# mueller-franzes/medfusion

Measured on AMD Instinct MI355X. Metric: images/sec at 256x256, 150 DDIM steps (DiffusionPipeline.sample incl. VAE decode), higher is better.
Workload: dtype f32 (emulated: fp16 pairs -- 23-bit operands, and 23-bit STORAGE of the tensors between the UNet's conv blocks: they exist as fp16 pairs only)

## Files before the change

### medfusion_amd/csrc/conv_f16x2.h

```cpp
#pragma once
#include "common.h"
#include "split_f16.h"

#ifndef MFC2_HZ
#define MFC2_HZ 0
#endif
#ifndef MFC2_OUT_STORE
#define MFC2_OUT_STORE 0
#endif

namespace mfc2 {
using namespace mf;

typedef float f32x16 __attribute__((ext_vector_type(16)));
typedef float f32x4 __attribute__((ext_vector_type(4)));
typedef unsigned int u32x4 __attribute__((ext_vector_type(4)));
typedef _Float16 f16x8 __attribute__((ext_vector_type(8)));
typedef _Float16 f16x2 __attribute__((ext_vector_type(2)));

struct FuseP {
  int on, act;
  float eps, bconst;
  double count;
  const float* gamma;
  const float* beta;
  const float* res_f32;
  const void* res_pairs;
  const float* res_bound;
  const float* res_slots;
  int res_nslots;
  int tiles_per_sample;
  const float* emb;
  long emb_stride;
  const float* emb_bound;
  float* out_f32;
  void* out_pairs;
  float* out_bound;
  unsigned* rv;
  unsigned* rv_err;
};

struct ConvP2 {
  const void* x1;
  const void* x2;
  const void* w;
  const float* bound1;
  const float* bound2;
  const float* bias;
  int N, Hin, Win, C1, C2, Cin, Cout;
  int Wout, Heff, Weff, KH, KW, stride, pad;
  int M, K, HWout;
  int cgroups, cg_per_split, splitk;
  int tiles_m, tiles_n;
  unsigned bytes1, bytes2, bytesw;
  int subpix, hw_src;
  int wphase_rows;
  int walk_n_fast;
  int tree;
  int wexp;
  int Hout;
  int bound_slots;
  int out_nt;
  float* y;
  float* out_bound;
  long slab;
  double* gn_partial;
  float* handoff;
  unsigned* sync;
  int gn_groups, gn_parts, gn_cpg;
  FuseP fz;
  float wl1_1, wl1_2;
  void* y_pairs;
  float* y_pair_bound;
  float bmax;
#if MFC2_HZ & (256 | 512)
  float* dbg;
#endif
};

static_assert(offsetof(ConvP2, wexp) == 168, "the ramp block: 6 pointers + 30 ints, nothing else in front of wexp");
static_assert(offsetof(ConvP2, gn_groups) - offsetof(ConvP2, wexp) <= 64 && offsetof(ConvP2, fz) + offsetof(FuseP, bconst) - offsetof(ConvP2, gn_groups) <= 64 &&
              offsetof(FuseP, res_nslots) - offsetof(FuseP, bconst) <= 64 && offsetof(FuseP, emb_stride) - offsetof(FuseP, res_nslots) <= 64 &&
              offsetof(ConvP2, wl1_1) - offsetof(ConvP2, fz) - offsetof(FuseP, emb_stride) <= 64 && offsetof(ConvP2, bmax) - offsetof(ConvP2, wl1_1) <= 64,
              "MFC2_RAMP_ARGS touches every 64-byte line of the epilogue's part");

#define MFC2_RAMP_ARGS(P)                                                                                               \
  __builtin_amdgcn_sched_barrier(0);    \
  asm volatile("" : "+s"(P.x1), "+s"(P.x2), "+s"(P.w), "+s"(P.bound1), "+s"(P.bound2), "+s"(P.bias), "+s"(P.N), "+s"(P.Hin), "+s"(P.Win), \
               "+s"(P.C1), "+s"(P.C2), "+s"(P.Cin), "+s"(P.Cout), "+s"(P.Wout));                                        \
  asm volatile("" : "+s"(P.Heff), "+s"(P.Weff), "+s"(P.KH), "+s"(P.KW), "+s"(P.stride), "+s"(P.pad), "+s"(P.M), "+s"(P.K), "+s"(P.HWout), \
               "+s"(P.cgroups), "+s"(P.cg_per_split), "+s"(P.splitk), "+s"(P.tiles_m), "+s"(P.tiles_n));                \
  asm volatile("" : "+s"(P.bytes1), "+s"(P.bytes2), "+s"(P.bytesw), "+s"(P.subpix), "+s"(P.hw_src), "+s"(P.wphase_rows), "+s"(P.walk_n_fast), \
               "+s"(P.tree)                                                                                             \
               : "s"(P.wexp), "s"(P.gn_groups), "s"(__float_as_int(P.fz.bconst)), "s"(P.fz.res_nslots), "s"((int)P.fz.emb_stride), "s"(__float_as_int(P.wl1_1)),   \
                 "s"(__float_as_int(P.bmax)));

__device__ __forceinline__ int xcd_remap2(int bid, int total) {
  const int q = total >> 3, r = total & 7;
  const int xcd = bid & 7, within = bid >> 3;
  const int base = xcd < r ? xcd * (q + 1) : r * (q + 1) + (xcd - r) * q;
  return base + within;
}

#ifndef MFC2_HZ
#define MFC2_HZ 0
#endif
#define MFC2_HZ_ON(BIT) ((MFC2_HZ >> (BIT)) & 1)
#ifndef MFC2_HZ_PAD
#define MFC2_HZ_PAD 7
#endif

__device__ __forceinline__ float hz_add(float a, float b) { float r; asm volatile("v_add_f32 %0, %1, %2" : "=v"(r) : "v"(a), "v"(b)); return r; }
__device__ __forceinline__ float hz_mul(float a, float b) { float r; asm volatile("v_mul_f32 %0, %1, %2" : "=v"(r) : "v"(a), "v"(b)); return r; }

#define MFC2_EPILOGUE_ARGS(OFF)                                                                                         \
  const char __attribute__((address_space(4)))* pk_ =                                                                   \
      (const char __attribute__((address_space(4)))*)__builtin_amdgcn_kernarg_segment_ptr() + (OFF);                    \
  asm volatile("" : "+s"(pk_));                                                                                         \
  const ConvP2& p = *(const ConvP2*)pk_;

#define MFC2_WAIT_VM(N) asm volatile("s_waitcnt vmcnt(%0)" ::"n"(N) : "memory")
#if MFC2_HZ & 512
#define MFC2_STAMP(I) { if (p.dbg && threadIdx.x == 0) reinterpret_cast<unsigned long*>(p.dbg)[(long)MFC2_BID * 8 + (I)] = __builtin_amdgcn_s_memrealtime(); }
#else
#define MFC2_STAMP(I)
#endif
#define MFC2_WAIT_LGKM0() asm volatile("s_waitcnt lgkmcnt(0)" ::: "memory")

#define MFC2_BODY_AS_KERNEL 1
#define MFC2_BID blockIdx.x
#define MFC2_KARG_OFF 0
#include "conv_f16x2_body.inc"
#undef MFC2_BODY_AS_KERNEL
#undef MFC2_BID
#undef MFC2_KARG_OFF
#define MFC2_BODY_AS_KERNEL 0
#define MFC2_BID bid
#define MFC2_KARG_OFF karg_off
#include "conv_f16x2_body.inc"
#undef MFC2_BODY_AS_KERNEL
#undef MFC2_BID
#undef MFC2_KARG_OFF

__global__ __launch_bounds__(256) void split_act_f16x2_kernel(const float* __restrict__ x, u32x4* __restrict__ out, long octets,
                                                              const float* __restrict__ bound, long octets_per_row) {
  const long stride = (long)gridDim.x * blockDim.x;
  for (long o = (long)blockIdx.x * blockDim.x + threadIdx.x; o < octets; o += stride) {
    const float sc = bound ? exp2i(-scale_exp_of(bound[o / octets_per_row])) : 1.f;
    const f32x4 v0 = *reinterpret_cast<const f32x4*>(x + o * 8) * sc, v1 = *reinterpret_cast<const f32x4*>(x + o * 8 + 4) * sc;
    u32x4 hi, lo;
    split8_f16(v0, v1, hi, lo);
    out[o * 2] = hi;
    out[o * 2 + 1] = lo;
  }
}

__global__ __launch_bounds__(256) void split_act_slots_kernel(const float* __restrict__ x, u32x4* __restrict__ out, long octets_per_row,
                                                              const float* __restrict__ slots, int nslots, float* __restrict__ bound_out) {
  __shared__ float sm[4];
  const int row = blockIdx.y, tid = threadIdx.x;
  float m = 0.f;
  for (int i = tid; i < nslots; i += 256) m = fmaxf(m, slots[(long)row * nslots + i]);
  m = mf::wave_max(m);
  if ((tid & 63) == 0) sm[tid >> 6] = m;
  __syncthreads();
  const float b = fmaxf(fmaxf(sm[0], sm[1]), fmaxf(sm[2], sm[3]));
  if (blockIdx.x == 0 && tid == 0) bound_out[row] = b;
  const float sc = exp2i(-scale_exp_of(b));
  const long base = (long)row * octets_per_row;
  for (long o = (long)blockIdx.x * 256 + tid; o < octets_per_row; o += (long)gridDim.x * 256) {
    const f32x4 v0 = *reinterpret_cast<const f32x4*>(x + (base + o) * 8) * sc, v1 = *reinterpret_cast<const f32x4*>(x + (base + o) * 8 + 4) * sc;
    u32x4 hi, lo;
    split8_f16(v0, v1, hi, lo);
    out[(base + o) * 2] = hi;
    out[(base + o) * 2 + 1] = lo;
  }
}

}
```

### medfusion_amd/csrc/conv_f16x2_epilogue.inc

```
  MFC2_WAIT_LGKM0();
  __builtin_amdgcn_s_barrier();
  MFC2_STAMP(4)
  if constexpr (MFC2_HZ_ON(0)) asm volatile("s_nop 15\n\ts_nop 15" ::: "memory");
  if (p.tree) {
#pragma unroll
    for (int i = 0; i < TM; ++i) {
      MFC2_PIXEL_EXPS(i)
      const float f_out = exp2i(last_src2 ? e2_ : e1_) * exp2i(p.wexp);
#pragma unroll
      for (int j = 0; j < TN; ++j)
#pragma unroll
        for (int r = 0; r < 16; ++r) { accm[i][j][r] = (accm[i][j][r] + accx[i][j][r] * kLoInv) * f_out; accx[i][j][r] = 0.f; }
    }
    constexpr int SLOT = BM * BN;
    const int tile = tile_n * p.tiles_m + tile_m;
    float* region = p.handoff + (long)tile * (2L * (p.splitk - 1)) * SLOT;
    const __amdgpu_buffer_rsrc_t rh = __builtin_amdgcn_make_buffer_rsrc(region, 0, (unsigned)(2 * (p.splitk - 1)) * (unsigned)SLOT * 4u, 0x00020000);
    unsigned* cnt = p.sync + (long)tile * (p.splitk - 1);
    unsigned* flag = reinterpret_cast<unsigned*>(smem);
    const unsigned lane_off = (unsigned)((wave * TM * TN * 4) * 64 + lane) * 16u;
    int lbase = 0;
    for (int span = 1; span < p.splitk; span <<= 1) {
      if constexpr (MFC2_HZ_ON(4)) asm volatile("s_nop 15" ::: "memory");
      const int lv = __builtin_ctz(span);
      const int side = (kz >> lv) & 1, pair = kz >> (lv + 1);
      const unsigned mine = (unsigned)(2 * (lbase + pair) + side) * (unsigned)SLOT * 4u, theirs = (unsigned)(2 * (lbase + pair) + (side ^ 1)) * (unsigned)SLOT * 4u;
#pragma unroll
      for (int i = 0; i < TM; ++i)
#pragma unroll
        for (int j = 0; j < TN; ++j)
#pragma unroll
          for (int q = 0; q < 4; ++q) {
            u32x4 v;
#pragma unroll
            for (int e = 0; e < 4; ++e) v[e] = __float_as_uint(accm[i][j][4 * q + e]);
            __builtin_amdgcn_raw_buffer_store_b128(v, rh, lane_off + (unsigned)(((i * TN + j) * 4 + q) * 1024), mine, 0x10);
          }
      MFC2_WAIT_VM(0);
      if constexpr (MFC2_HZ_ON(4)) asm volatile("s_nop 15" ::: "memory");
      __syncthreads();
      if (tid == 0) {
        if (p.tree == 2) {
          __builtin_amdgcn_fence(__ATOMIC_RELEASE, "agent");
          MFC2_WAIT_VM(0);
        }
        const unsigned old = __hip_atomic_fetch_add(cnt + lbase + pair, 1u, __ATOMIC_RELAXED, __HIP_MEMORY_SCOPE_AGENT);
        if (old) __hip_atomic_store(cnt + lbase + pair, 0u, __ATOMIC_RELAXED, __HIP_MEMORY_SCOPE_AGENT);
        if (p.tree == 2 && old) __builtin_amdgcn_fence(__ATOMIC_ACQUIRE, "agent");
        *flag = old;
      }
      __syncthreads();
      const unsigned second = *flag;
      __syncthreads();
      if (!second) return;
      if constexpr (MFC2_HZ_ON(3)) {
        u32x4 pv[TM * TN * 4];
#pragma unroll
        for (int u = 0; u < TM * TN * 4; ++u) pv[u] = __builtin_amdgcn_raw_buffer_load_b128(rh, lane_off + (unsigned)(u * 1024), theirs, 0x10);
        asm volatile("s_waitcnt vmcnt(0)\n\ts_nop 7" ::: "memory");
#if MFC2_HZ & 256
        if (p.dbg) {
          const long plane = (long)p.tiles_m * p.tiles_n * NW * (TM * TN * 16 * 64);
          float* o = p.dbg + ((long)tile * NW + wave) * (TM * TN * 16 * 64) + lane;
#pragma unroll
          for (int u = 0; u < TM * TN * 4; ++u)
#pragma unroll
            for (int e = 0; e < 4; ++e) {
              __builtin_nontemporal_store(accm[u / (4 * TN)][(u / 4) % TN][4 * (u % 4) + e], o + plane + (u * 4 + e) * 64);
              __builtin_nontemporal_store(__uint_as_float(pv[u][e]), o + 2 * plane + (u * 4 + e) * 64);
            }
        }
#endif
#pragma unroll
        for (int u = 0; u < TM * TN * 4; ++u)
#pragma unroll
          for (int e = 0; e < 4; ++e) accm[u / (4 * TN)][(u / 4) % TN][4 * (u % 4) + e] += __uint_as_float(pv[u][e]);
      } else {
#pragma unroll
      for (int i = 0; i < TM; ++i)
#pragma unroll
        for (int j = 0; j < TN; ++j)
#pragma unroll
          for (int q = 0; q < 4; ++q) {
            const u32x4 v = __builtin_amdgcn_raw_buffer_load_b128(rh, lane_off + (unsigned)(((i * TN + j) * 4 + q) * 1024), theirs, 0x10);
#pragma unroll
            for (int e = 0; e < 4; ++e) {
              if constexpr (MFC2_HZ_ON(5)) accm[i][j][4 * q + e] = hz_add(accm[i][j][4 * q + e], __uint_as_float(v[e]));
              else accm[i][j][4 * q + e] += __uint_as_float(v[e]);
            }
          }
      }
      lbase += p.splitk >> (lv + 1);
    }
#if MFC2_HZ & 256
    if (p.dbg) {
      float* o = p.dbg + ((long)tile * NW + wave) * (TM * TN * 16 * 64) + lane;
#pragma unroll
      for (int i = 0; i < TM; ++i)
#pragma unroll
        for (int j = 0; j < TN; ++j)
#pragma unroll
          for (int r = 0; r < 16; ++r) __builtin_nontemporal_store(accm[i][j][r], o + ((i * TN + j) * 16 + r) * 64);
    }
#endif
  }
  MFC2_STAMP(5)
  const bool last_slice = p.splitk == 1 || p.tree;
  constexpr int PITCH = FN * 4 + 16;
  char* stg = smem + wave * (32 * PITCH);
  static_assert(NW * 32 * PITCH <= MFC2_EPILOGUE_LDS_BYTES, "epilogue staging must fit in the pipeline stages");
  constexpr int LPR = FN / 8, RPP = 64 / LPR, NPASS = 32 / RPP;
  const int rr = lane / LPR, c8 = lane % LPR;
  const int col0 = n0 + wn * FN + c8 * 8;
  float* out = p.y + (last_slice ? 0L : (long)kz * p.slab);
#if MFC2_OUT_STORE == 2
  const __amdgpu_buffer_rsrc_t rs_out = __builtin_amdgcn_make_buffer_rsrc(out, 0, (unsigned)((long)p.M * p.Cout * 4), 0x00020000);
#endif
#if MFC2_EXPS_EARLY
  f32x4 b0 = eb0, b1 = eb1;
  asm volatile("" : "+v"(b0), "+v"(b1));
#else
  f32x4 b0 = {0.f, 0.f, 0.f, 0.f}, b1 = {0.f, 0.f, 0.f, 0.f};
  if (last_slice && p.bias) {
    b0 = *reinterpret_cast<const f32x4*>(p.bias + col0);
    b1 = *reinterpret_cast<const f32x4*>(p.bias + col0 + 4);
  }
#endif
  float s1 = 0.f, s2 = 0.f, vmax = 0.f;
  const bool fz = p.fz.on != 0;
  f32x4 yk0[TM][NPASS], yk1[TM][NPASS];
#pragma unroll
  for (int i = 0; i < TM; ++i) {
    MFC2_PIXEL_EXPS(i)
    const float f_out = p.tree ? 1.f : exp2i(last_src2 ? e2_ : e1_) * exp2i(p.wexp);
#pragma unroll
    for (int j = 0; j < TN; ++j)
#pragma unroll
      for (int q = 0; q < 4; ++q) {
        f32x4 v;
#pragma unroll
        for (int e = 0; e < 4; ++e) {
          if constexpr (MFC2_HZ_ON(6)) v[e] = hz_mul(hz_add(accm[i][j][4 * q + e], hz_mul(accx[i][j][4 * q + e], kLoInv)), f_out);
          else v[e] = (accm[i][j][4 * q + e] + accx[i][j][4 * q + e] * kLoInv) * f_out;
        }
        *reinterpret_cast<f32x4*>(stg + (lane & 31) * PITCH + (j * 32 + 8 * q + 4 * fh) * 4) = v;
        if constexpr (MFC2_HZ_ON(7)) asm volatile("s_nop 0" ::: "memory");
        if constexpr (MFC2_HZ_ON(1)) asm volatile("s_nop %1" : "+v"(v) : "n"(MFC2_HZ_PAD) : "memory");
      }
    f32x4 rv0[NPASS], rv1[NPASS];
#pragma unroll
    for (int ps = 0; ps < NPASS; ++ps) {
      rv0[ps] = *reinterpret_cast<const f32x4*>(stg + (ps * RPP + rr) * PITCH + c8 * 32);
      rv1[ps] = *reinterpret_cast<const f32x4*>(stg + (ps * RPP + rr) * PITCH + c8 * 32 + 16);
    }
#pragma unroll
    for (int ps = 0; ps < NPASS; ++ps) {
      const int row = ps * RPP + rr;
      f32x4 v0 = rv0[ps], v1 = rv1[ps];
      if constexpr (MFC2_HZ_ON(2)) asm volatile("s_waitcnt lgkmcnt(0)\n\ts_nop 3" : "+v"(v0), "+v"(v1)::"memory");
      v0 += b0;
      v1 += b1;
      const int m = m0 + wm * FM + i * 32 + row;
      yk0[i][ps] = v0;
      yk1[i][ps] = v1;
      if (fz) {
        if (m < p.M) {
#pragma unroll
          for (int e = 0; e < 4; ++e) {
            s1 += v0[e] + v1[e];
            s2 = fmaf(v0[e], v0[e], s2);
            s2 = fmaf(v1[e], v1[e], s2);
          }
        }
      } else if (m < p.M) {
        long orow = m;
        if (p.subpix) {
          const int n = m / p.HWout, rem = m - n * p.HWout;
          const int ph = rem / p.hw_src, r2 = rem - ph * p.hw_src;
          const int y = r2 / p.Win, x = r2 - y * p.Win;
          orow = ((long)n * p.Hout + 2 * y + (ph >> 1)) * p.Wout + 2 * x + (ph & 1);
        }
#if MFC2_OUT_STORE == 1
        __builtin_nontemporal_store(v0, reinterpret_cast<f32x4*>(out + orow * p.Cout + col0));
        __builtin_nontemporal_store(v1, reinterpret_cast<f32x4*>(out + orow * p.Cout + col0 + 4));
#elif MFC2_OUT_STORE == 2
        {
          const unsigned ob_ = (unsigned)((orow * p.Cout + col0) * 4);
          __builtin_amdgcn_raw_buffer_store_b128(__builtin_bit_cast(u32x4, v0), rs_out, ob_, 0, 0x10);
          __builtin_amdgcn_raw_buffer_store_b128(__builtin_bit_cast(u32x4, v1), rs_out, ob_ + 16u, 0, 0x10);
        }
#else
        if (p.out_nt) {
          __builtin_nontemporal_store(v0, reinterpret_cast<f32x4*>(out + orow * p.Cout + col0));
          __builtin_nontemporal_store(v1, reinterpret_cast<f32x4*>(out + orow * p.Cout + col0 + 4));
        } else {
          *reinterpret_cast<f32x4*>(out + orow * p.Cout + col0) = v0;
          *reinterpret_cast<f32x4*>(out + orow * p.Cout + col0 + 4) = v1;
        }
#endif
        if (p.out_bound) {
#pragma unroll
          for (int e = 0; e < 4; ++e) vmax = fmaxf(vmax, fmaxf(fabsf(v0[e]), fabsf(v1[e])));
        }
        if (p.y_pairs) {
          const int nrow = m / p.HWout;
          const float yb = p.bound1[nrow] * p.wl1_1 + (p.C2 > 0 ? p.bound2[nrow] * p.wl1_2 : 0.f) + p.bmax;
          const float ysc = exp2i(-scale_exp_of(yb));
          sf_u32x4 hi, lo;
          split8_f16<false>(v0 * ysc, v1 * ysc, hi, lo);
          sf_u32x4* op = reinterpret_cast<sf_u32x4*>(reinterpret_cast<char*>(p.y_pairs) + ((orow * p.Cout + col0) >> 3) * 32);
          op[0] = hi;
          op[1] = lo;
          if (m - nrow * p.HWout == 0 && col0 == 0) p.y_pair_bound[nrow] = yb;
        }
#pragma unroll
        for (int e = 0; e < 4; ++e) {
          s1 += v0[e] + v1[e];
          s2 = fmaf(v0[e], v0[e], s2);
          s2 = fmaf(v1[e], v1[e], s2);
        }
      }
    }
  }
  MFC2_STAMP(6)
  const int wm_per_sample = p.HWout >= BM ? WM : p.HWout / FM;
  const int n_first = m0 / p.HWout;
  if (p.out_bound) {
    vmax = wave_max(vmax);
    const int n = n_first + wm / wm_per_sample;
    const int part = p.HWout >= BM ? (m0 - n_first * p.HWout) / BM : 0;
    const int wps = wm_per_sample * WN;
    if (lane == 0 && n < p.N) p.out_bound[(long)n * p.bound_slots + (part * p.tiles_n + tile_n) * wps + (wm % wm_per_sample) * WN + wn] = vmax;
  }
  if (p.gn_partial) {
    double d1 = (double)s1, d2 = (double)s2;
#pragma unroll
    for (int off = LPR; off < 64; off <<= 1) {
      d1 += __shfl_xor(d1, off, 64);
      d2 += __shfl_xor(d2, off, 64);
    }
    __builtin_amdgcn_s_barrier();
    double* red = reinterpret_cast<double*>(smem);
    if (lane < LPR) {
      red[(wave * LPR + lane) * 2] = d1;
      red[(wave * LPR + lane) * 2 + 1] = d2;
    }
    MFC2_WAIT_LGKM0();
    __builtin_amdgcn_s_barrier();
    const int ngl = BN / p.gn_cpg, spt = WM / wm_per_sample;
    if (tid < ngl * spt) {
      const int gl = tid % ngl, si = tid / ngl;
      double s = 0, q = 0;
      const int slots = p.gn_cpg >> 3;
      for (int k = 0; k < slots; ++k) {
        const int slot8 = gl * slots + k;
        const int wn_ = slot8 / LPR, c8_ = slot8 - wn_ * LPR;
        for (int wm_ = si * wm_per_sample; wm_ < (si + 1) * wm_per_sample; ++wm_) {
          const double* d = red + ((wm_ * WN + wn_) * LPR + c8_) * 2;
          s += d[0];
          q += d[1];
        }
      }
      const int n = n_first + si;
      const int part = p.HWout >= BM ? (m0 - n_first * p.HWout) / BM : 0;
      if (n < p.N) {
        double* o = p.gn_partial + (((long)n * p.gn_parts + part) * p.gn_groups + (n0 / p.gn_cpg + gl)) * 2;
        if (fz) {
          __hip_atomic_store(o, s, __ATOMIC_RELAXED, __HIP_MEMORY_SCOPE_AGENT);
          __hip_atomic_store(o + 1, q, __ATOMIC_RELAXED, __HIP_MEMORY_SCOPE_AGENT);
        } else {
          o[0] = s;
          o[1] = q;
        }
      }
    }
  }
  if (fz) {
    MFC2_WAIT_VM(0);
    __syncthreads();
    const int spt = WM / wm_per_sample;
    const int ngl_ = BN / p.gn_cpg;
    const unsigned T_ = (unsigned)p.fz.tiles_per_sample;
    if (tid == 0) {
      for (int si = 0; si < spt; ++si) {
        const int n = n_first + si;
        if (n < p.N) __hip_atomic_fetch_add(p.fz.rv + 2 * n, 1u, __ATOMIC_RELAXED, __HIP_MEMORY_SCOPE_AGENT);
      }
    }
    MFC2_STAMP(6)
    const int si_w = wm / wm_per_sample;
    const int n_w = min(n_first + si_w, p.N - 1);
    float* fzs = reinterpret_cast<float*>(smem + 8192);
    float rb = 0.f;
    if (p.fz.res_slots) {
      for (int si = 0; si < spt; ++si) {
        const int n = min(n_first + si, p.N - 1);
        float mx = 0.f;
        for (int k = tid; k < p.fz.res_nslots; k += NW * 64) mx = fmaxf(mx, p.fz.res_slots[(long)n * p.fz.res_nslots + k]);
        mx = wave_max(mx);
        if (lane == 0) fzs[si * 8 + wave] = mx;
      }
      MFC2_WAIT_LGKM0();
      __syncthreads();
#pragma unroll
      for (int w8 = 0; w8 < NW; ++w8) rb = fmaxf(rb, fzs[si_w * 8 + w8]);
    } else if (p.fz.res_bound) {
      rb = p.fz.res_bound[n_w];
    }
    const float ob_ = p.fz.bconst + rb + (p.fz.emb_bound ? p.fz.emb_bound[n_w] : 0.f);
    const float osc = exp2i(-scale_exp_of(ob_));
    const float rsc = p.fz.res_pairs ? exp2i(scale_exp_of(p.fz.res_bound[n_w])) : 1.f;
    {
      const int part0 = p.HWout >= BM ? (m0 - n_first * p.HWout) / BM : 0;
      if (tile_n == 0 && part0 == 0 && wn == 0 && (wm % wm_per_sample) == 0 && lane == 0 && n_first + si_w < p.N) p.fz.out_bound[n_first + si_w] = ob_;
    }
    f32x4 ga0 = {1.f, 1.f, 1.f, 1.f}, ga1 = ga0, be0 = {0.f, 0.f, 0.f, 0.f}, be1 = be0, em0 = be0, em1 = be0;
    if (p.fz.gamma) {
      ga0 = *reinterpret_cast<const f32x4*>(p.fz.gamma + col0); ga1 = *reinterpret_cast<const f32x4*>(p.fz.gamma + col0 + 4);
      be0 = *reinterpret_cast<const f32x4*>(p.fz.beta + col0);  be1 = *reinterpret_cast<const f32x4*>(p.fz.beta + col0 + 4);
    }
    if (p.fz.emb) {
      const float* er = p.fz.emb + (long)n_w * p.fz.emb_stride + col0;
      em0 = *reinterpret_cast<const f32x4*>(er); em1 = *reinterpret_cast<const f32x4*>(er + 4);
    }
    f32x4 rk0[TM][NPASS], rk1[TM][NPASS];
#pragma unroll
    for (int i = 0; i < TM; ++i)
#pragma unroll
      for (int ps = 0; ps < NPASS; ++ps) {
        const int m = m0 + wm * FM + i * 32 + ps * RPP + rr;
        rk0[i][ps] = f32x4{0.f, 0.f, 0.f, 0.f};
        rk1[i][ps] = f32x4{0.f, 0.f, 0.f, 0.f};
        if (m < p.M) {
          const long e = (long)m * p.Cout + col0;
          if (p.fz.res_pairs) {
            const f32x4* g = reinterpret_cast<const f32x4*>(reinterpret_cast<const char*>(p.fz.res_pairs) + (e >> 3) * 32);
            rk0[i][ps] = g[0]; rk1[i][ps] = g[1];
          } else if (p.fz.res_f32) {
            rk0[i][ps] = *reinterpret_cast<const f32x4*>(p.fz.res_f32 + e); rk1[i][ps] = *reinterpret_cast<const f32x4*>(p.fz.res_f32 + e + 4);
          }
        }
      }
    if (tid == 0) {
      unsigned ok = 1u;
      for (int si = 0; si < spt; ++si) {
        const int n = n_first + si;
        if (n >= p.N) continue;
        const unsigned long t0 = __builtin_amdgcn_s_memrealtime();
        unsigned spins = 0;
        while (__hip_atomic_load(p.fz.rv + 2 * n, __ATOMIC_RELAXED, __HIP_MEMORY_SCOPE_AGENT) < T_) {
          __builtin_amdgcn_s_sleep(1);
          if ((++spins & 127u) == 0u) {
            if (__hip_atomic_load(p.fz.rv_err, __ATOMIC_RELAXED, __HIP_MEMORY_SCOPE_AGENT) != 0u) { ok = 0u; break; }
            if (__builtin_amdgcn_s_memrealtime() - t0 > 5000000ul) {
              __hip_atomic_store(p.fz.rv_err, 1u, __ATOMIC_RELAXED, __HIP_MEMORY_SCOPE_AGENT);
              ok = 0u;
              break;
            }
          }
        }
      }
      reinterpret_cast<unsigned*>(fzs)[64] = ok;
    }
    MFC2_WAIT_LGKM0();
    __syncthreads();
    MFC2_STAMP(7)
    if (tid < ngl_ * spt) {
      const int gl = tid % ngl_, si = tid / ngl_;
      const int n = n_first + si;
      if (n < p.N) {
        const int G_ = p.gn_groups, PPT = 256 / G_, g = n0 / p.gn_cpg + gl;
        double S = 0, Q = 0;
        for (int kk = 0; kk < PPT; ++kk) {
          double a = 0, b = 0;
          for (int k = kk; k < p.gn_parts; k += PPT) {
            const double* r_ = p.gn_partial + (((long)n * p.gn_parts + k) * G_ + g) * 2;
            a += __hip_atomic_load(r_, __ATOMIC_RELAXED, __HIP_MEMORY_SCOPE_AGENT);
            b += __hip_atomic_load(r_ + 1, __ATOMIC_RELAXED, __HIP_MEMORY_SCOPE_AGENT);
          }
          if (kk == 0) { S = a; Q = b; } else { S += a; Q += b; }
        }
        const double mean = S / p.fz.count;
        double var = Q / p.fz.count - mean * mean;
        if (var < 0) var = 0;
        fzs[128 + (si * ngl_ + gl) * 2] = (float)mean;
        fzs[128 + (si * ngl_ + gl) * 2 + 1] = (float)(1.0 / sqrt(var + (double)p.fz.eps));
      }
    }
    MFC2_WAIT_LGKM0();
    __syncthreads();
    if (tid == 0) {
      for (int si = 0; si < spt; ++si) {
        const int n = n_first + si;
        if (n >= p.N) continue;
        const unsigned old = __hip_atomic_fetch_add(p.fz.rv + 2 * n + 1, 1u, __ATOMIC_RELAXED, __HIP_MEMORY_SCOPE_AGENT);
        if (old + 1u == T_) {
          __hip_atomic_store(p.fz.rv + 2 * n, 0u, __ATOMIC_RELAXED, __HIP_MEMORY_SCOPE_AGENT);
          __hip_atomic_store(p.fz.rv + 2 * n + 1, 0u, __ATOMIC_RELAXED, __HIP_MEMORY_SCOPE_AGENT);
        }
      }
    }
    const int glw = (wn * FN + c8 * 8) / p.gn_cpg;
    const float mean_ = fzs[128 + (si_w * ngl_ + glw) * 2], rstd_ = fzs[128 + (si_w * ngl_ + glw) * 2 + 1];
    const bool aff = p.fz.gamma != nullptr, act1 = p.fz.act == 1, resp = p.fz.res_pairs != nullptr, resf = !resp && p.fz.res_f32 != nullptr,
               hasemb = p.fz.emb != nullptr;
#pragma unroll
    for (int i = 0; i < TM; ++i)
#pragma unroll
      for (int ps = 0; ps < NPASS; ++ps) {
        const int m = m0 + wm * FM + i * 32 + ps * RPP + rr;
        if (m < p.M) {
          float ev[8];
#pragma unroll
          for (int e = 0; e < 4; ++e) { ev[e] = yk0[i][ps][e]; ev[4 + e] = yk1[i][ps][e]; }
          const float gv[8] = {ga0[0], ga0[1], ga0[2], ga0[3], ga1[0], ga1[1], ga1[2], ga1[3]};
          const float bv[8] = {be0[0], be0[1], be0[2], be0[3], be1[0], be1[1], be1[2], be1[3]};
          const float mv[8] = {em0[0], em0[1], em0[2], em0[3], em1[0], em1[1], em1[2], em1[3]};
#pragma unroll
          for (int e = 0; e < 8; ++e) {
            float t = (ev[e] - mean_) * rstd_;
            if (aff) t = t * gv[e] + bv[e];
            if (act1) t = swish_apply(t);
            ev[e] = t;
          }
          if (resp) {
            const u32x4 hq = __builtin_bit_cast(u32x4, rk0[i][ps]), lq = __builtin_bit_cast(u32x4, rk1[i][ps]);
#pragma unroll
            for (int e2 = 0; e2 < 4; ++e2) {
              const unsigned hw_ = hq[e2], lw_ = lq[e2];
              const f16x2 h2 = __builtin_bit_cast(f16x2, hw_), l2 = __builtin_bit_cast(f16x2, lw_);
              ev[2 * e2] += ((float)h2[0] + (float)l2[0] * kLoInv) * rsc;
              ev[2 * e2 + 1] += ((float)h2[1] + (float)l2[1] * kLoInv) * rsc;
            }
          } else if (resf) {
#pragma unroll
            for (int e = 0; e < 4; ++e) { ev[e] += rk0[i][ps][e]; ev[4 + e] += rk1[i][ps][e]; }
          }
          if (hasemb) {
#pragma unroll
            for (int e = 0; e < 8; ++e) ev[e] += mv[e];
          }
          const long eo = (long)m * p.Cout + col0;
          if (p.fz.out_f32) {
            *reinterpret_cast<f32x4*>(p.fz.out_f32 + eo) = f32x4{ev[0], ev[1], ev[2], ev[3]};
            *reinterpret_cast<f32x4*>(p.fz.out_f32 + eo + 4) = f32x4{ev[4], ev[5], ev[6], ev[7]};
          }
          sf_u32x4 hi, lo;
          split8_f16<false>(sf_f32x4{ev[0] * osc, ev[1] * osc, ev[2] * osc, ev[3] * osc}, sf_f32x4{ev[4] * osc, ev[5] * osc, ev[6] * osc, ev[7] * osc}, hi, lo);
          sf_u32x4* op = reinterpret_cast<sf_u32x4*>(reinterpret_cast<char*>(p.fz.out_pairs) + (eo >> 3) * 32);
          op[0] = hi;
          op[1] = lo;
        }
      }
  }
```

Baseline: 43.05.

## Restructure conv epilogue drain: preload kernargs, batch LDS staging, prefetch pair bounds

Before the epilogue barrier, the conv epilogue now copies the kernel arguments it uses into scalar/vector registers and preloads the per-row pair-bound values. It stages all TM row-groups through LDS at once when they fit, so the reads are batched instead of serialized per group. Global stores use explicit address_space(1) pointers, and the y_pair_bound writes move to a separate pass after the loop. The aim is to shorten the dependent scalar-load and LDS chains in the drain, at the cost of more registers (pyb/pyn/rv arrays) and possibly lower occupancy.

```diff
diff --git a/medfusion_amd/csrc/conv_f16x2.h b/medfusion_amd/csrc/conv_f16x2.h
--- a/medfusion_amd/csrc/conv_f16x2.h
+++ b/medfusion_amd/csrc/conv_f16x2.h
@@ -113,6 +113,9 @@
 __device__ __forceinline__ float hz_add(float a, float b) { float r; asm volatile("v_add_f32 %0, %1, %2" : "=v"(r) : "v"(a), "v"(b)); return r; }
 __device__ __forceinline__ float hz_mul(float a, float b) { float r; asm volatile("v_mul_f32 %0, %1, %2" : "=v"(r) : "v"(a), "v"(b)); return r; }
 
+#ifndef MFC2_DRAIN_CHAIN
+#define MFC2_DRAIN_CHAIN 2
+#endif
 #define MFC2_EPILOGUE_ARGS(OFF)                                                                                         \
   const char __attribute__((address_space(4)))* pk_ =                                                                   \
       (const char __attribute__((address_space(4)))*)__builtin_amdgcn_kernarg_segment_ptr() + (OFF);                    \
diff --git a/medfusion_amd/csrc/conv_f16x2_epilogue.inc b/medfusion_amd/csrc/conv_f16x2_epilogue.inc
--- a/medfusion_amd/csrc/conv_f16x2_epilogue.inc
+++ b/medfusion_amd/csrc/conv_f16x2_epilogue.inc
@@ -1,12 +1,53 @@
+#if MFC2_DRAIN_CHAIN == 2
+  int dp_M = p.M, dp_Cout = p.Cout, dp_HWout = p.HWout, dp_subpix = p.subpix, dp_out_nt = p.out_nt,
+      dp_fz_on = p.fz.on, dp_hw_src = p.hw_src, dp_Win = p.Win, dp_Hout = p.Hout, dp_Wout = p.Wout;
+  float *dp_y = p.y, *dp_out_bound = p.out_bound;
+  void* dp_y_pairs = p.y_pairs;
+  __builtin_amdgcn_sched_barrier(0);
+  asm volatile("" : "+s"(dp_M), "+s"(dp_Cout), "+s"(dp_HWout), "+s"(dp_subpix), "+s"(dp_out_nt), "+s"(dp_fz_on),
+               "+s"(dp_y), "+s"(dp_out_bound), "+s"(dp_y_pairs));
+  asm volatile("" : "+v"(dp_hw_src), "+v"(dp_Win), "+v"(dp_Hout), "+v"(dp_Wout));
+#define MFC2_G(T, P) ((T __attribute__((address_space(1)))*)(P))
+#define MFC2_DP_SET(F) (dp_##F != nullptr)
+#define dp_slab p.slab
+#define dp_tree p.tree
+#define dp_wexp p.wexp
+#define dp_splitk p.splitk
+#define dp_gn_partial p.gn_partial
+#define MFC2_DP(F) dp_##F
+#else
+#define MFC2_DP(F) p.F
+#define MFC2_DP_SET(F) (p.F != nullptr)
+#define MFC2_G(T, P) (reinterpret_cast<T*>(P))
+#define dp_fz_on p.fz.on
+#endif
+#if MFC2_DRAIN_CHAIN == 2
+  float pyb1[TM][32 / (64 / (FN / 8))] = {}, pyb2[TM][32 / (64 / (FN / 8))] = {};
+  int pyn[TM][32 / (64 / (FN / 8))] = {};
+  float* ypb_ = nullptr;
+  if (MFC2_DP_SET(y_pairs)) {
+    ypb_ = p.y_pair_bound;
+    const float* pb2_ = p.C2 > 0 ? p.bound2 : p.bound1;
+#pragma unroll
+    for (int i = 0; i < TM; ++i)
+#pragma unroll
+      for (int ps = 0; ps < 32 / (64 / (FN / 8)); ++ps) {
+        const int nrow = min(m0 + wm * FM + i * 32 + ps * (64 / (FN / 8)) + lane / (FN / 8), MFC2_DP(M) - 1) / MFC2_DP(HWout);
+        pyn[i][ps] = nrow;
+        pyb1[i][ps] = p.bound1[nrow];
+        pyb2[i][ps] = pb2_[nrow];
+      }
+  }
+#endif
   MFC2_WAIT_LGKM0();
   __builtin_amdgcn_s_barrier();
   MFC2_STAMP(4)
   if constexpr (MFC2_HZ_ON(0)) asm volatile("s_nop 15\n\ts_nop 15" ::: "memory");
-  if (p.tree) {
+  if (MFC2_DP(tree)) {
 #pragma unroll
     for (int i = 0; i < TM; ++i) {
       MFC2_PIXEL_EXPS(i)
-      const float f_out = exp2i(last_src2 ? e2_ : e1_) * exp2i(p.wexp);
+      const float f_out = exp2i(last_src2 ? e2_ : e1_) * exp2i(MFC2_DP(wexp));
 #pragma unroll
       for (int j = 0; j < TN; ++j)
 #pragma unroll
@@ -14,13 +55,13 @@
     }
     constexpr int SLOT = BM * BN;
     const int tile = tile_n * p.tiles_m + tile_m;
-    float* region = p.handoff + (long)tile * (2L * (p.splitk - 1)) * SLOT;
-    const __amdgpu_buffer_rsrc_t rh = __builtin_amdgcn_make_buffer_rsrc(region, 0, (unsigned)(2 * (p.splitk - 1)) * (unsigned)SLOT * 4u, 0x00020000);
-    unsigned* cnt = p.sync + (long)tile * (p.splitk - 1);
+    float* region = p.handoff + (long)tile * (2L * (MFC2_DP(splitk) - 1)) * SLOT;
+    const __amdgpu_buffer_rsrc_t rh = __builtin_amdgcn_make_buffer_rsrc(region, 0, (unsigned)(2 * (MFC2_DP(splitk) - 1)) * (unsigned)SLOT * 4u, 0x00020000);
+    unsigned* cnt = p.sync + (long)tile * (MFC2_DP(splitk) - 1);
     unsigned* flag = reinterpret_cast<unsigned*>(smem);
     const unsigned lane_off = (unsigned)((wave * TM * TN * 4) * 64 + lane) * 16u;
     int lbase = 0;
-    for (int span = 1; span < p.splitk; span <<= 1) {
+    for (int span = 1; span < MFC2_DP(splitk); span <<= 1) {
       if constexpr (MFC2_HZ_ON(4)) asm volatile("s_nop 15" ::: "memory");
       const int lv = __builtin_ctz(span);
       const int side = (kz >> lv) & 1, pair = kz >> (lv + 1);
@@ -40,13 +81,13 @@
       if constexpr (MFC2_HZ_ON(4)) asm volatile("s_nop 15" ::: "memory");
       __syncthreads();
       if (tid == 0) {
-        if (p.tree == 2) {
+        if (MFC2_DP(tree) == 2) {
           __builtin_amdgcn_fence(__ATOMIC_RELEASE, "agent");
           MFC2_WAIT_VM(0);
         }
         const unsigned old = __hip_atomic_fetch_add(cnt + lbase + pair, 1u, __ATOMIC_RELAXED, __HIP_MEMORY_SCOPE_AGENT);
         if (old) __hip_atomic_store(cnt + lbase + pair, 0u, __ATOMIC_RELAXED, __HIP_MEMORY_SCOPE_AGENT);
-        if (p.tree == 2 && old) __builtin_amdgcn_fence(__ATOMIC_ACQUIRE, "agent");
+        if (MFC2_DP(tree) == 2 && old) __builtin_amdgcn_fence(__ATOMIC_ACQUIRE, "agent");
         *flag = old;
       }
       __syncthreads();
@@ -90,7 +131,7 @@
             }
           }
       }
-      lbase += p.splitk >> (lv + 1);
+      lbase += MFC2_DP(splitk) >> (lv + 1);
     }
 #if MFC2_HZ & 256
     if (p.dbg) {
@@ -105,16 +146,18 @@
 #endif
   }
   MFC2_STAMP(5)
-  const bool last_slice = p.splitk == 1 || p.tree;
+  const bool last_slice = MFC2_DP(splitk) == 1 || MFC2_DP(tree);
   constexpr int PITCH = FN * 4 + 16;
-  char* stg = smem + wave * (32 * PITCH);
-  static_assert(NW * 32 * PITCH <= MFC2_EPILOGUE_LDS_BYTES, "epilogue staging must fit in the pipeline stages");
+  constexpr int GI = (MFC2_DRAIN_CHAIN == 2 && NW * TM * 32 * PITCH <= MFC2_EPILOGUE_LDS_BYTES) ? TM : 1;
+  constexpr int STG = GI * 32 * PITCH;
+  char* stg = smem + wave * STG;
+  static_assert(NW * STG <= MFC2_EPILOGUE_LDS_BYTES, "epilogue staging must fit in the pipeline stages");
   constexpr int LPR = FN / 8, RPP = 64 / LPR, NPASS = 32 / RPP;
   const int rr = lane / LPR, c8 = lane % LPR;
   const int col0 = n0 + wn * FN + c8 * 8;
-  float* out = p.y + (last_slice ? 0L : (long)kz * p.slab);
+  float* out = MFC2_DP(y) + (last_slice ? 0L : (long)kz * MFC2_DP(slab));
 #if MFC2_OUT_STORE == 2
-  const __amdgpu_buffer_rsrc_t rs_out = __builtin_amdgcn_make_buffer_rsrc(out, 0, (unsigned)((long)p.M * p.Cout * 4), 0x00020000);
+  const __amdgpu_buffer_rsrc_t rs_out = __builtin_amdgcn_make_buffer_rsrc(out, 0, (unsigned)((long)MFC2_DP(M) * MFC2_DP(Cout) * 4), 0x00020000);
 #endif
 #if MFC2_EXPS_EARLY
   f32x4 b0 = eb0, b1 = eb1;
@@ -127,12 +170,15 @@
   }
 #endif
   float s1 = 0.f, s2 = 0.f, vmax = 0.f;
-  const bool fz = p.fz.on != 0;
+  const bool fz = dp_fz_on != 0;
   f32x4 yk0[TM][NPASS], yk1[TM][NPASS];
-#pragma unroll
-  for (int i = 0; i < TM; ++i) {
+  f32x4 rv0[TM][NPASS], rv1[TM][NPASS];
+#pragma unroll
+  for (int g = 0; g < TM; g += GI) {
+#pragma unroll
+  for (int i = g; i < g + GI; ++i) {
     MFC2_PIXEL_EXPS(i)
-    const float f_out = p.tree ? 1.f : exp2i(last_src2 ? e2_ : e1_) * exp2i(p.wexp);
+    const float f_out = MFC2_DP(tree) ? 1.f : exp2i(last_src2 ? e2_ : e1_) * exp2i(MFC2_DP(wexp));
 #pragma unroll
     for (int j = 0; j < TN; ++j)
 #pragma unroll
@@ -143,20 +189,41 @@
           if constexpr (MFC2_HZ_ON(6)) v[e] = hz_mul(hz_add(accm[i][j][4 * q + e], hz_mul(accx[i][j][4 * q + e], kLoInv)), f_out);
           else v[e] = (accm[i][j][4 * q + e] + accx[i][j][4 * q + e] * kLoInv) * f_out;
         }
-        *reinterpret_cast<f32x4*>(stg + (lane & 31) * PITCH + (j * 32 + 8 * q + 4 * fh) * 4) = v;
+        *reinterpret_cast<f32x4*>(stg + (i - g) * (32 * PITCH) + (lane & 31) * PITCH + (j * 32 + 8 * q + 4 * fh) * 4) = v;
         if constexpr (MFC2_HZ_ON(7)) asm volatile("s_nop 0" ::: "memory");
         if constexpr (MFC2_HZ_ON(1)) asm volatile("s_nop %1" : "+v"(v) : "n"(MFC2_HZ_PAD) : "memory");
       }
-    f32x4 rv0[NPASS], rv1[NPASS];
+  }
+#pragma unroll
+  for (int i = g; i < g + GI; ++i) {
 #pragma unroll
     for (int ps = 0; ps < NPASS; ++ps) {
-      rv0[ps] = *reinterpret_cast<const f32x4*>(stg + (ps * RPP + rr) * PITCH + c8 * 32);
-      rv1[ps] = *reinterpret_cast<const f32x4*>(stg + (ps * RPP + rr) * PITCH + c8 * 32 + 16);
-    }
+      rv0[i][ps] = *reinterpret_cast<const f32x4*>(stg + (i - g) * (32 * PITCH) + (ps * RPP + rr) * PITCH + c8 * 32);
+      rv1[i][ps] = *reinterpret_cast<const f32x4*>(stg + (i - g) * (32 * PITCH) + (ps * RPP + rr) * PITCH + c8 * 32 + 16);
+    }
+  }
+#if MFC2_DRAIN_CHAIN == 2
+  if (g == 0) {
+#pragma unroll
+    for (int i = 0; i < TM; ++i)
+#pragma unroll
+      for (int ps = 0; ps < NPASS; ++ps) asm volatile("" : "+v"(pyb1[i][ps]), "+v"(pyb2[i][ps]));
+    asm volatile("" : "+v"(ypb_));
+    const float wl1_1 = p.wl1_1, wl1_2 = p.wl1_2, bmax = p.bmax;
+    const bool src2 = p.C2 > 0;
+#pragma unroll
+    for (int i = 0; i < TM; ++i)
+#pragma unroll
+      for (int ps = 0; ps < NPASS; ++ps)
+        pyb1[i][ps] = pyb1[i][ps] * wl1_1 + (src2 ? pyb2[i][ps] * wl1_2 : 0.f) + bmax;
+  }
+#endif
+#pragma unroll
+  for (int i = g; i < g + GI; ++i) {
 #pragma unroll
     for (int ps = 0; ps < NPASS; ++ps) {
       const int row = ps * RPP + rr;
-      f32x4 v0 = rv0[ps], v1 = rv1[ps];
+      f32x4 v0 = rv0[i][ps], v1 = rv1[i][ps];
       if constexpr (MFC2_HZ_ON(2)) asm volatile("s_waitcnt lgkmcnt(0)\n\ts_nop 3" : "+v"(v0), "+v"(v1)::"memory");
       v0 += b0;
       v1 += b1;
@@ -164,7 +231,7 @@
       yk0[i][ps] = v0;
       yk1[i][ps] = v1;
       if (fz) {
-        if (m < p.M) {
+        if (m < MFC2_DP(M)) {
 #pragma unroll
           for (int e = 0; e < 4; ++e) {
             s1 += v0[e] + v1[e];
@@ -172,46 +239,52 @@
             s2 = fmaf(v1[e], v1[e], s2);
           }
         }
-      } else if (m < p.M) {
+      } else if (m < MFC2_DP(M)) {
         long orow = m;
-        if (p.subpix) {
-          const int n = m / p.HWout, rem = m - n * p.HWout;
-          const int ph = rem / p.hw_src, r2 = rem - ph * p.hw_src;
-          const int y = r2 / p.Win, x = r2 - y * p.Win;
-          orow = ((long)n * p.Hout + 2 * y + (ph >> 1)) * p.Wout + 2 * x + (ph & 1);
+        if (MFC2_DP(subpix)) {
+          const int n = m / MFC2_DP(HWout), rem = m - n * MFC2_DP(HWout);
+          const int ph = rem / MFC2_DP(hw_src), r2 = rem - ph * MFC2_DP(hw_src);
+          const int y = r2 / MFC2_DP(Win), x = r2 - y * MFC2_DP(Win);
+          orow = ((long)n * MFC2_DP(Hout) + 2 * y + (ph >> 1)) * MFC2_DP(Wout) + 2 * x + (ph & 1);
         }
 #if MFC2_OUT_STORE == 1
-        __builtin_nontemporal_store(v0, reinterpret_cast<f32x4*>(out + orow * p.Cout + col0));
-        __builtin_nontemporal_store(v1, reinterpret_cast<f32x4*>(out + orow * p.Cout + col0 + 4));
+        __builtin_nontemporal_store(v0, MFC2_G(f32x4, out + orow * MFC2_DP(Cout) + col0));
+        __builtin_nontemporal_store(v1, MFC2_G(f32x4, out + orow * MFC2_DP(Cout) + col0 + 4));
 #elif MFC2_OUT_STORE == 2
         {
-          const unsigned ob_ = (unsigned)((orow * p.Cout + col0) * 4);
+          const unsigned ob_ = (unsigned)((orow * MFC2_DP(Cout) + col0) * 4);
           __builtin_amdgcn_raw_buffer_store_b128(__builtin_bit_cast(u32x4, v0), rs_out, ob_, 0, 0x10);
           __builtin_amdgcn_raw_buffer_store_b128(__builtin_bit_cast(u32x4, v1), rs_out, ob_ + 16u, 0, 0x10);
         }
 #else
-        if (p.out_nt) {
-          __builtin_nontemporal_store(v0, reinterpret_cast<f32x4*>(out + orow * p.Cout + col0));
-          __builtin_nontemporal_store(v1, reinterpret_cast<f32x4*>(out + orow * p.Cout + col0 + 4));
+        if (MFC2_DP(out_nt)) {
+          __builtin_nontemporal_store(v0, MFC2_G(f32x4, out + orow * MFC2_DP(Cout) + col0));
+          __builtin_nontemporal_store(v1, MFC2_G(f32x4, out + orow * MFC2_DP(Cout) + col0 + 4));
         } else {
-          *reinterpret_cast<f32x4*>(out + orow * p.Cout + col0) = v0;
-          *reinterpret_cast<f32x4*>(out + orow * p.Cout + col0 + 4) = v1;
-        }
-#endif
-        if (p.out_bound) {
+          *MFC2_G(f32x4, out + orow * MFC2_DP(Cout) + col0) = v0;
+          *MFC2_G(f32x4, out + orow * MFC2_DP(Cout) + col0 + 4) = v1;
+        }
+#endif
+        if (MFC2_DP_SET(out_bound)) {
 #pragma unroll
           for (int e = 0; e < 4; ++e) vmax = fmaxf(vmax, fmaxf(fabsf(v0[e]), fabsf(v1[e])));
         }
-        if (p.y_pairs) {
-          const int nrow = m / p.HWout;
+        if (MFC2_DP_SET(y_pairs)) {
+#if MFC2_DRAIN_CHAIN == 2
+          const float yb = pyb1[i][ps];
+#else
+          const int nrow = m / MFC2_DP(HWout);
           const float yb = p.bound1[nrow] * p.wl1_1 + (p.C2 > 0 ? p.bound2[nrow] * p.wl1_2 : 0.f) + p.bmax;
+#endif
           const float ysc = exp2i(-scale_exp_of(yb));
           sf_u32x4 hi, lo;
           split8_f16<false>(v0 * ysc, v1 * ysc, hi, lo);
-          sf_u32x4* op = reinterpret_cast<sf_u32x4*>(reinterpret_cast<char*>(p.y_pairs) + ((orow * p.Cout + col0) >> 3) * 32);
+          auto op = MFC2_G(sf_u32x4, reinterpret_cast<char*>(MFC2_DP(y_pairs)) + ((orow * MFC2_DP(Cout) + col0) >> 3) * 32);
           op[0] = hi;
           op[1] = lo;
-          if (m - nrow * p.HWout == 0 && col0 == 0) p.y_pair_bound[nrow] = yb;
+#if MFC2_DRAIN_CHAIN != 2
+          if (m - nrow * MFC2_DP(HWout) == 0 && col0 == 0) MFC2_DP(y_pair_bound)[nrow] = yb;
+#endif
         }
 #pragma unroll
         for (int e = 0; e < 4; ++e) {
@@ -222,17 +295,34 @@
       }
     }
   }
+  }
+#if MFC2_DRAIN_CHAIN == 2
+  if (!fz && MFC2_DP_SET(y_pairs)) {
+    auto ypb = MFC2_G(float, ypb_);
+#pragma unroll
+    for (int i = 0; i < TM; ++i)
+#pragma unroll
+      for (int ps = 0; ps < NPASS; ++ps) {
+        const int m = m0 + wm * FM + i * 32 + ps * RPP + rr;
+        if (m < MFC2_DP(M) && m - pyn[i][ps] * MFC2_DP(HWout) == 0 && col0 == 0) ypb[pyn[i][ps]] = pyb1[i][ps];
+      }
+  }
+#endif
   MFC2_STAMP(6)
-  const int wm_per_sample = p.HWout >= BM ? WM : p.HWout / FM;
-  const int n_first = m0 / p.HWout;
-  if (p.out_bound) {
+  const int wm_per_sample = MFC2_DP(HWout) >= BM ? WM : MFC2_DP(HWout) / FM;
+#if MFC2_DRAIN_CHAIN == 2
+  const int n_first = (int)((unsigned)m0 / (unsigned)MFC2_DP(HWout));
+#else
+  const int n_first = m0 / MFC2_DP(HWout);
+#endif
+  if (MFC2_DP_SET(out_bound)) {
     vmax = wave_max(vmax);
     const int n = n_first + wm / wm_per_sample;
-    const int part = p.HWout >= BM ? (m0 - n_first * p.HWout) / BM : 0;
+    const int part = MFC2_DP(HWout) >= BM ? (m0 - n_first * MFC2_DP(HWout)) / BM : 0;
     const int wps = wm_per_sample * WN;
-    if (lane == 0 && n < p.N) p.out_bound[(long)n * p.bound_slots + (part * p.tiles_n + tile_n) * wps + (wm % wm_per_sample) * WN + wn] = vmax;
-  }
-  if (p.gn_partial) {
+    if (lane == 0 && n < p.N) MFC2_G(float, MFC2_DP(out_bound))[(long)n * p.bound_slots + (part * p.tiles_n + tile_n) * wps + (wm % wm_per_sample) * WN + wn] = vmax;
+  }
+  if (MFC2_DP(gn_partial)) {
     double d1 = (double)s1, d2 = (double)s2;
 #pragma unroll
     for (int off = LPR; off < 64; off <<= 1) {
@@ -262,9 +352,9 @@
         }
       }
       const int n = n_first + si;
-      const int part = p.HWout >= BM ? (m0 - n_first * p.HWout) / BM : 0;
+      const int part = MFC2_DP(HWout) >= BM ? (m0 - n_first * MFC2_DP(HWout)) / BM : 0;
       if (n < p.N) {
-        double* o = p.gn_partial + (((long)n * p.gn_parts + part) * p.gn_groups + (n0 / p.gn_cpg + gl)) * 2;
+        double* o = MFC2_DP(gn_partial) + (((long)n * p.gn_parts + part) * p.gn_groups + (n0 / p.gn_cpg + gl)) * 2;
         if (fz) {
           __hip_atomic_store(o, s, __ATOMIC_RELAXED, __HIP_MEMORY_SCOPE_AGENT);
           __hip_atomic_store(o + 1, q, __ATOMIC_RELAXED, __HIP_MEMORY_SCOPE_AGENT);
@@ -453,3 +543,15 @@
         }
       }
   }
+#undef MFC2_DP
+#undef MFC2_DP_SET
+#undef MFC2_G
+#if MFC2_DRAIN_CHAIN == 2
+#undef dp_slab
+#undef dp_tree
+#undef dp_wexp
+#undef dp_splitk
+#undef dp_gn_partial
+#else
+#undef dp_fz_on
+#endif
```

Result: no change. 43.06 (median of 2 runs) (+0.0%).
